# CaptainEven/DenseBox

Measured on AMD Instinct MI355X. Metric: training patches/sec (240x240), higher is better.
Workload: dtype f16; 1 GPU; full training step (fwd + fused dense loss w/ hard-negative mining + bwd + grad all-reduce + SGD) of DenseBoxLMLOC on 240x240 patches; net=DenseBoxLMLOC, batch_per_gpu=64, global_batch=64, patch=240x240, parallelism=dp1, half_neg=11, grad_finite=True

## Files before the change

densebox_amd/_lib.py:

```python
import ctypes as C
import os

_HERE = os.path.dirname(os.path.abspath(__file__))
LIB_PATH = os.environ.get('DBX_LIB') or os.path.join(_HERE, 'csrc', 'libdensebox_hip.so')

F16, BF16, F32 = 0, 1, 2
DTYPE_ID = {'f16': F16, 'bf16': BF16, 'f32': F32}
ESIZE = {F16: 2, BF16: 2, F32: 4}

EPI_BIAS, EPI_RELU, EPI_GATE, EPI_DROPMASK, EPI_ACCUM, EPI_F32_NCHW, EPI_DROPHASH = 1, 2, 4, 8, 16, 32, 64
CONV_WFRAG = 128
K_IGEMM, K_DMA, K_BAND, K_C64, K_C8, K_WS, K_P8 = 1, 2, 3, 4, 5, 6, 7


class View(C.Structure):
    _fields_ = [('ptr', C.c_void_p), ('n', C.c_int32), ('h', C.c_int32), ('w', C.c_int32),
                ('pad', C.c_int32), ('ld', C.c_int32), ('c_off', C.c_int32), ('c', C.c_int32)]


class ConvDesc(C.Structure):
    _fields_ = [('dtype', C.c_int32), ('kh', C.c_int32), ('kw', C.c_int32), ('cpad', C.c_int32),
                ('cin_pad', C.c_int32), ('cout_pad', C.c_int32), ('epilogue', C.c_int32), ('drop_seed', C.c_uint32)]


# ... 169 lines not shown
    'dbx_conv_forward': (C.c_int, [_PC, _PV, _VP, _VP, _PV, _PV, _VP, _I32, _VP]),
    'dbx_conv_plan': (C.c_int, [_PC, _PV, _PV, C.POINTER(ConvPlan)]),
    'dbx_conv_forward_split': (C.c_int, [_PC, _PV, _VP, _VP, _PV, _PV, _PV, _PV, _I32, _I32, _VP]),
    'dbx_heads_forward_fusable': (C.c_int, [_PC, _PV, _PV, C.POINTER(C.c_int32), _I32]),
    'dbx_heads_forward_fused_scratch_bytes': (_I64, [_I32, _I64]),
    'dbx_heads_forward_fused': (C.c_int, [_PC, _PV, _VP, _VP, _PV, _VP, _VP, C.POINTER(C.c_int32), _I32, _VP, _VP, _VP]),
    'dbx_heads_forward_fused_heads': (C.c_int, [_PC, _PV, _VP, _VP, _PV, _VP, _VP, C.POINTER(C.c_int32), _I32, C.POINTER(C.c_void_p), _VP, _VP]),
    'dbx_dp_unique_id': (C.c_int, [_VP]),
    'dbx_dp_init': (C.c_int, [_VP, _I32, _I32, C.POINTER(C.c_void_p)]),
    'dbx_dp_allreduce_sum_f32': (C.c_int, [_VP, _VP, _I64, _VP]),
    'dbx_dp_destroy': (C.c_int, [_VP]),
    'dbx_conv_dgrad_wgrad1_scratch_bytes': (_I64, []),
    'dbx_conv_dgrad_wgrad1_fusable': (C.c_int, [_PC, _PV, _PV, _PV]),
    'dbx_conv_dgrad_wgrad1': (C.c_int, [_PC, _PV, _VP, _PV, _PV, _I32, _VP, _VP, _VP, _I32, _VP]),
    'dbx_conv_pool_fusable': (C.c_int, [_PC, _PV, _PV]),
    'dbx_conv_forward_pool': (C.c_int, [_PC, _PV, _VP, _VP, _PV, _PV, _I32, _VP]),
    'dbx_conv_forward_pool_idx': (C.c_int, [_PC, _PV, _VP, _VP, _PV, _PV, _I32, _VP, _VP]),
    'dbx_pack_weight': (C.c_int, [_I32, _I32, _VP, _I32, _I32, _I32, _I32, _VP, _I32, _I32, _I32, _I32, _VP]),
    'dbx_fold_heads': (C.c_int, [_VP, _VP, _VP, _VP, _I32, _VP, _VP, _VP]),
    'dbx_fold_refine': (C.c_int, [_VP, _VP, _VP, _VP, _VP, _VP, _I32, _I32, _VP, _VP, _VP, _VP]),
    'dbx_refine_eval': (C.c_int, [_VP, _VP, _I32, _I32, _I32, _VP, _VP, _VP, _VP]),
    'dbx_refine_backward_scratch_bytes': (C.c_int64, [_I32, _I32, _I32]),
    'dbx_refine_backward': (C.c_int, [_VP, _VP, _VP, _I32, _I32, _I32, _VP, _VP, _VP, _VP, _VP, _VP, _I32, _VP, _VP, _VP, _VP, _VP, _VP, _VP, _VP, _VP, _VP, _VP, _VP, _VP, _VP]),
    'dbx_upsample_bilinear_nchw_f32': (C.c_int, [_VP, _I32, _I32, _I32, _VP, _I32, _I32, _VP]),
    'dbx_pack_multi': (C.c_int, [_I32, _VP, _I32, _I64, _VP]),
    'dbx_sgd_pack_step': (C.c_int, [_I32, _VP, _I32, _I64, _VP, _F, _F, _F, _I32, _VP]),
    'dbx_head2_dgrad': (C.c_int, [_I32, _PV, C.POINTER(C.c_void_p), C.POINTER(C.c_int32), _I32, _PV, _VP, _I32, _I32, C.c_uint32, _VP]),
    'dbx_head2_wgrad_scratch_bytes': (_I64, [_I32, _I32]),
    'dbx_head2_wgrad': (C.c_int, [_I32, _PV, _PV, C.POINTER(C.c_int32), _I32, C.POINTER(C.c_void_p), C.POINTER(C.c_void_p), _VP, _VP]),
    'dbx_head2_backward': (C.c_int, [_I32, _PV, _PV, C.POINTER(C.c_void_p), C.POINTER(C.c_int32), _I32, _PV, _VP, _I32, _I32, C.c_uint32,
                                     C.POINTER(C.c_void_p), C.POINTER(C.c_void_p), _VP, _VP]),
    'dbx_head2_backward_up': (C.c_int, [_I32, _PV, _PV, C.POINTER(C.c_void_p), C.POINTER(C.c_int32), _I32, _PV, _VP, _I32, _I32, C.c_uint32,
                                        C.POINTER(C.c_void_p), C.POINTER(C.c_void_p), _VP, _PV, _VP]),
    'dbx_perspective_matrix': (C.c_int, [_VP, _VP, _VP]),
    'dbx_warp_perspective_u8': (C.c_int, [_VP, _I32, _I32, _I32, _VP, _VP, _I32, _I32, _VP]),
    'dbx_warp_batch_workspace_bytes': (_I64, [_I32]),
    'dbx_warp_perspective_batch_u8': (C.c_int, [C.POINTER(WarpJob), _I32, _I32, _VP, _VP, _VP]),
    'dbx_plate_crops_batch': (C.c_int, [_VP, _I32, _I32, _VP, _I64, _I64, _VP, _I32, _I32, _I32, _VP, _VP, _VP, _VP]),
    'dbx_match_gt_batch': (C.c_int, [_VP, _I32, _I64, _VP, _VP, _I32, _I32, _VP, _I32, _VP, _VP, _I32, _D, _VP, _VP, _VP, _VP, _VP, _VP]),
    'dbx_eval_append': (C.c_int, [_VP, _I32, _I64, _VP, _VP, _I32, _I32, _VP, _VP, _VP, _VP, _I64, _VP, _VP]),
    'dbx_track_update_batch': (C.c_int, [_VP, _I32, _I64, _VP, _VP, _I32, _I32, _VP, _VP, _I32, _I32, _I32, _D, _I32, _D, _D, _D, _VP, _VP, _VP,
                                         _VP, _VP, _VP]),
    'dbx_track_append': (C.c_int, [_VP, _VP, _I32, _I32, _I32, _VP, _I64, _VP, _VP]),
    'dbx_crop_sharpness': (C.c_int, [_VP, _I64, _I32, _I32, _I32, _VP, _VP]),
    'dbx_track_gallery_update': (C.c_int, [_VP, _VP, _VP, _VP, _VP, _VP, _VP, _VP, _VP, _VP, _VP, _VP, _VP, _I32, _I32, _I32, _I32, _I32, _I32,
                                           _I32, _I32, _I64, _I32, _D, _I32, _VP]),
    'dbx_draw_overlay_batch': (C.c_int, [_VP, _I32, _I32, _I32, _I32, _VP, _I32, _I64, _VP, _VP, _I32, _VP, _VP, _VP, _I32, _I32,
                                         C.POINTER(OverlayStyle), _VP]),
    'dbx_overlay_font': (C.c_int, [_VP]),
    'dbx_overlay_label': (C.c_int, [_D, _I32, C.c_char_p, _I32]),
    'dbx_redact_batch': (C.c_int, [_VP, _I32, _I32, _I32, _I32, _VP, _I32, _I64, _VP, _VP, _I32, _VP, _I32, _I32, _I32,
                                   C.POINTER(RedactStyle), _VP]),
    'dbx_redact_host': (C.c_int, [_VP, _VP, _I32, _I32, _I32, _VP, _I32, _I32, _VP, _I32, _VP, _I32, C.POINTER(RedactStyle)]),
    'dbx_resize_batch_workspace_bytes': (_I64, [_I32]),
    'dbx_resize_cubic_batch_u8': (C.c_int, [C.POINTER(ResizeJob), _I32, _I32, _VP, _VP, _VP]),
    'dbx_nv12_to_rgb_batch': (C.c_int, [_VP, _I32, _I32, _I32, C.POINTER(Nv12Params), _VP]),
    'dbx_rgb_to_nv12_batch': (C.c_int, [_VP, _I32, _I32, _I32, C.POINTER(Nv12Params), _VP]),
    'dbx_nv12_host': (C.c_int, [C.POINTER(Nv12Frame), C.POINTER(Nv12Params), _I32]),
    'dbx_resize_batch_nv12_workspace_bytes': (_I64, [_I32]),
    'dbx_resize_cubic_batch_nv12': (C.c_int, [C.POINTER(ResizeJobNv12), _I32, C.POINTER(Nv12Params), _VP, _VP, _VP]),
    'dbx_patch_plan': (C.c_int, [C.POINTER(PatchPlanIO), _I32, _I32, _I32, _I32, _I32, _D, _D, _I32, _VP]),
    'dbx_patch_cut': (C.c_int, [_VP, _VP, _I32, _I32, _VP, _VP]),
    'dbx_patch_plan_host': (C.c_int, [_I32, _I32, _I32, _VP, _I32, _D, _D, _D, _I32, C.POINTER(PatchGeom)]),
    'dbx_patch_draw': (C.c_int, [_I64, _I64, _I32, _I32, _VP]),
    'dbx_patch_check_tables': (C.c_int, [_VP, _I32, _VP, _I32, _VP, _I32]),
    'dbx_patch_aug_plan': (C.c_int, [C.POINTER(PatchAugIO), C.POINTER(PatchAugCfg), _I32, _VP]),
# ... 104 lines not shown
```

densebox_amd/csrc/aux_ops.hip:

```cpp
#include "common.hpp"
#include <mutex>

static thread_local char g_err[512] = "";
void dbx_set_error(const char* fmt, ...) {
    va_list ap;
    va_start(ap, fmt);
    vsnprintf(g_err, sizeof(g_err), fmt, ap);
    va_end(ap);
}
extern "C" const char* dbx_last_error(void) { return g_err; }
extern "C" int dbx_version(void) { return DBX_ABI_VERSION; }
extern "C" int dbx_device_arch(int device) {
    hipDeviceProp_t p;
    if (hipGetDeviceProperties(&p, device) != hipSuccess) { dbx_set_error("hipGetDeviceProperties failed"); return DBX_ERR_HIP; }
    int arch = 0;
    const char* s = p.gcnArchName;
    if (s[0] == 'g' && s[1] == 'f' && s[2] == 'x') arch = (int)strtol(s + 3, nullptr, 16) == 0x950 ? 950 : (int)strtol(s + 3, nullptr, 10);
    return arch;
}

template <typename T> struct Vec { static constexpr int N = 16 / sizeof(T); };

template <typename T> __device__ __forceinline__ void load_vec(const T* p, float (&v)[16 / sizeof(T)]) {
    const u32x4 raw = *(const u32x4*)p;
// ... 1438 lines not shown
extern "C" int dbx_head2_backward_up_plan(int32_t dtype, const dbx_view* hid, const dbx_view* d_g44, const int32_t* k, int32_t nh,
                                          dbx_head2_up_plan_t* out) {
    if (!hid || !d_g44 || !k || !out) { dbx_set_error("head2_backward_up_plan: null argument"); return DBX_ERR_ARG; }
    if (dtype != DBX_F16 && dtype != DBX_BF16 && dtype != DBX_F32) { dbx_set_error("head2_backward_up_plan: unknown dtype"); return DBX_ERR_DTYPE; }
    DBX_REQUIRE(nh >= 1 && nh <= 4 && hid->c == 512 * nh && d_g44->n == hid->n && d_g44->c == hid->c,
                "head2_backward_up_plan: nh in 1..4, hid of 512*nh channels, d_g44 with the hidden map's batch and channels");
    for (int i = 0; i < nh; ++i) DBX_REQUIRE(k[i] >= 1 && k[i] <= 8, "head2_backward_up_plan: k in 1..8");
    *out = dbx_head2_up_plan_t{};
    float sy, sx;
    H2UPlan plan;
    if (!h2u_fused(dtype == DBX_F32 ? 4 : 2, hid, d_g44, sy, sx, plan)) return DBX_OK;
    out->fused = 1; out->halves = plan.halves;
    for (int i = 0; i < 2; ++i) {
        const H2UHalf& h = plan.h[i];
        out->half[i].px_lo = h.px_lo; out->half[i].px_n = h.px_n; out->half[i].own_lo = h.own_lo; out->half[i].own_hi = h.own_hi;
        out->half[i].ix_lo = h.ix_lo; out->half[i].ix_n = h.ix_n;
    }
    H2ULaunch l[4];
    out->launches = h2u_launches(k, nh, hid->n, plan.halves, l);
    for (int i = 0; i < out->launches; ++i) {
        out->launch[i].head0 = l[i].h0; out->launch[i].heads = l[i].nhl; out->launch[i].kj = l[i].kj; out->launch[i].groups = l[i].groups;
        out->launch[i].blocks = l[i].blocks;
    }
    return DBX_OK;
}
extern "C" int dbx_head2_backward_up(int32_t dtype, const dbx_view* d_out, const dbx_view* hid, const float* const* w2, const int32_t* k,
                                     int32_t nh, const dbx_view* d_hid, const uint8_t* dropmask, int32_t dropmask_ld, int32_t use_hash,
                                     uint32_t drop_seed, float* const* dw, float* const* db, void* scratch, const dbx_view* d_g44, void* stream) {
    if (!d_out || !hid || !w2 || !k || !d_hid || !dw || !scratch || !d_g44) { dbx_set_error("head2_backward_up: null argument"); return DBX_ERR_ARG; }
    DBX_DISPATCH_DTYPE(dtype, head2_backward_up_t, d_out, hid, w2, k, nh, d_hid, dropmask, dropmask_ld, use_hash, (unsigned)drop_seed, dw, db,
                       scratch, d_g44, (hipStream_t)stream);
}

struct PackJob { const float* src; void* dst; int co, ci, taps, mode; long long ktot; int cin_pad, row_off, k_off, rows_lim; };
template <typename T>
__global__ void pack_multi_kernel(const PackJob* __restrict__ jobs) {
    const PackJob j = jobs[blockIdx.y];
    const int total = j.co * j.ci * j.taps, taps = j.taps, ci = j.ci;
    T* wp = (T*)j.dst;
    const bool fwd = j.mode == 0 || j.mode == 4;
    const int rl = j.mode >= 4 ? (int)j.ktot : j.rows_lim;
    if (sizeof(T) == 2 && j.mode != 2 && (fwd ? ci : j.co) % 8 == 0 && (j.k_off & 7) == 0 && (j.cin_pad & 7) == 0 && taps <= 25) {
        __shared__ float tile[8][32 * 25];
        const int ot = (j.co + 7) / 8, ctn = (ci + 31) / 32, ntiles = ot * ctn, row_f = 32 * taps;
        for (int tl = blockIdx.x; tl < ntiles; tl += gridDim.x) {
            const int o0 = (tl / ctn) * 8, c0 = (tl % ctn) * 32;
            const int cw = min(32, ci - c0), ow = min(8, j.co - o0);
            __syncthreads();
            for (int e = threadIdx.x; e < 8 * row_f; e += blockDim.x) {
                const int r = e / row_f, f = e - r * row_f;
                tile[r][f] = (r < ow && f < cw * taps) ? j.src[((o0 + r) * ci + c0) * taps + f] : 0.f;
            }
            __syncthreads();
            const int nch = fwd ? 8 * taps * 4 : 32 * taps;
            for (int q = threadIdx.x; q < nch; q += blockDim.x) {
                int row, col, tap;
                float v[8];
                if (fwd) {
                    const int k8 = q & 3, t = (q >> 2) % taps, r = (q >> 2) / taps;
                    if (r >= ow || 8 * k8 >= cw) continue;
                    row = j.row_off + o0 + r; col = j.k_off + c0 + 8 * k8; tap = t;
#pragma unroll
                    for (int e = 0; e < 8; ++e) v[e] = tile[r][(8 * k8 + e) * taps + t];
                } else {
                    const int c = q % 32, t = q / 32;
                    if (c >= cw) continue;
// ... 358 lines not shown
```

densebox_amd/engine.py:

```python
import collections
import contextlib
import ctypes as C
import os
import weakref

import torch

from . import _lib
from ._lib import View, ConvDesc, check, ptr, stream_ptr

_BACKBONE = [('conv1_1_1', 3, 64), ('conv1_2_1', 64, 64), ('conv2_1_1', 64, 128), ('conv2_2_1', 128, 128),
             ('conv3_1_1', 128, 256), ('conv3_2_1', 256, 256), ('conv3_4_1', 256, 256),
             ('conv4_1_1', 256, 512), ('conv4_2_1', 512, 512), ('conv4_3_1', 512, 512), ('conv4_4_1', 512, 512)]

_HEADS = {
    'DenseBox': [('det', 1), ('loc', 4)],
    'DenseBoxLM': [('det', 1), ('loc', 4), ('landmark', 4)],
    'DenseBoxLMLOC': [('det', 1), ('loc', 4), ('landmark', 4), ('lmloc', 8)],
}


_FWD_IO = {'conv1_1_1': ('x0', 'a11'), 'conv1_2_1': ('a11', 'a12'), 'conv2_1_1': ('p1', 'a21'), 'conv2_2_1': ('a21', 'a22'),
           'conv3_1_1': ('p2', 'a31'), 'conv3_2_1': ('a31', 'a32'), 'conv3_4_1': ('a32', 'c34'), 'conv4_1_1': ('p3', 'a41'),
           'conv4_2_1': ('a41', 'a42'), 'conv4_3_1': ('a42', 'a43'), 'conv4_4_1': ('a43', 'a44')}
# ... 904 lines not shown
        for i, (stem, k) in enumerate(heads):
            slot[stem] = B['d_out'].view(P.crf * i, P.crf)
            src = override.get(stem)
            srcs.append(src if src is not None else gout(stem, k))
        if override or kind == 'DenseBox':
            check(L.dbx_nchw_to_framed_slots(dt, (C.c_void_p * nh)(*[t.data_ptr() for t in srcs]), (C.c_int32 * nh)(*[k for _, k in heads]), nh, P.crf,
                                             C.byref(B['d_out'].view()), s))
        else:
            for (stem, k), t in zip(heads, srcs):
                check(L.dbx_nchw_to_framed(dt, ptr(t), k, C.byref(slot[stem]), s))
        if kind != 'DenseBox' and not override:
            check(L.dbx_framed_add_ch(dt, C.byref(B['d_rf_in'].view()), 0, 4, C.byref(slot['landmark']), 0, s))
            check(L.dbx_framed_add_ch(dt, C.byref(B['d_rf_in'].view()), 4, 1, C.byref(slot['det']), 0, s))

        hv = B['hid'].view()
        need = L.dbx_head2_wgrad_scratch_bytes(nh, hv.n * hv.h)
        if getattr(self, '_h2_scratch', None) is None or self._h2_scratch.numel() < need:
            self._h2_scratch = torch.empty(int(need), dtype=torch.uint8, device=dev)
        dw2 = [new_grad('conv5_2_%s.weight' % st) for st, _ in heads]
        db2 = [new_grad('conv5_2_%s.bias' % st) for st, _ in heads]
        w2s = [self._param('conv5_2_%s.weight' % st).detach() for st, _ in heads]
        ks = (C.c_int32 * nh)(*[k for _, k in heads])
        h2_names = ['conv5_2_%s.weight' % st for st, _ in heads] + ['conv5_2_%s.bias' % st for st, _ in heads]
        mask_p = C.c_void_p(P.mask_buf.data_ptr()) if (P.drop_active and not P.drop_hash) else None
        hash_on, hash_seed = (1 if P.drop_hash else 0), (P.drop_seed if P.drop_hash else 0)
        lin = ('heads1', 'bwd_a') in M
        up_done = False
        gen = bool(getattr(P, 'heads_gen', False) and lin and side is None and mask_p is None)
        if gen and dt != _lib.F32:
            dhid_v = View(None, hv.n, hv.h, hv.w, 1, 512 * nh, 0, 512 * nh)
        else:
            dhid_v = self._d_hid(P).view()
        w2p = (C.c_void_p * nh)(*[w.data_ptr() for w in w2s])
        with self._timed(lambda: ('head2_backward_up_kernel<%s>' if up_done else 'head2_wgrad_kernel<%s>') % _TNAME[dt],
                         2.0 * hv.n * hv.h * hv.w * 512 * sum(k for _, k in heads) * (1 if side is not None else 2)):
            if side is not None:
                def run_h2():
                    check(L.dbx_head2_wgrad(dt, C.byref(B['d_out'].view()), C.byref(hv), ks, nh,
                                            (C.c_void_p * nh)(*[t.data_ptr() for t in dw2]), (C.c_void_p * nh)(*[t.data_ptr() for t in db2]),
                                            ptr(self._h2_scratch), stream_ptr()))
                    if sink is not None:
                        sink.ready(h2_names)
                on_side(run_h2)
                check(L.dbx_head2_dgrad(dt, C.byref(B['d_out'].view()), (C.c_void_p * nh)(*[w.data_ptr() for w in w2s]), ks, nh,
                                        C.byref(dhid_v), mask_p, 512 * nh, hash_on, hash_seed, s))
            elif lin:
                check(L.dbx_head2_backward_up(dt, C.byref(B['d_out'].view()), C.byref(hv), (C.c_void_p * nh)(*[w.data_ptr() for w in w2s]), ks, nh,
                                              C.byref(dhid_v), mask_p, 512 * nh, hash_on, hash_seed,
                                              (C.c_void_p * nh)(*[t.data_ptr() for t in dw2]), (C.c_void_p * nh)(*[t.data_ptr() for t in db2]),
                                              ptr(self._h2_scratch), C.byref(B['d_g44'].view()), s))
                up_done = True
                if gen and dt == _lib.F32:
                    bh = P.B['d_hid']
                    P.ws[bh.off:bh.off + bh.bytes].view(torch.float32).fill_(float('nan'))
            else:
                check(L.dbx_head2_backward(dt, C.byref(B['d_out'].view()), C.byref(hv), (C.c_void_p * nh)(*[w.data_ptr() for w in w2s]), ks, nh,
                                           C.byref(dhid_v), mask_p, 512 * nh, hash_on, hash_seed,
                                           (C.c_void_p * nh)(*[t.data_ptr() for t in dw2]), (C.c_void_p * nh)(*[t.data_ptr() for t in db2]),
                                           ptr(self._h2_scratch), s))
                if sink is not None:
                    sink.ready(h2_names)
        w1n = ['conv5_1_%s.weight' % st for st, _ in heads]
        b1n = ['conv5_1_%s.bias' % st for st, _ in heads]
        if sink is not None:
            dw1, db1 = sink.region(w1n).view(512 * nh, 768, 1, 1), sink.region(b1n)
        else:
            dw1 = torch.empty((512 * nh, 768, 1, 1), dtype=torch.float32, device=dev)
            db1 = torch.empty((512 * nh,), dtype=torch.float32, device=dev)
        c34 = B['fusion'].view(512, 256)
# ... 114 lines not shown
```

include/densebox_hip.h:

```cpp
#ifndef DENSEBOX_HIP_H
#define DENSEBOX_HIP_H

#include <stdint.h>

#ifdef __cplusplus
extern "C" {
#endif

enum dbx_status {
    DBX_OK = 0,
    DBX_ERR_ARG = -1,
    DBX_ERR_HIP = -2,
    DBX_ERR_DTYPE = -3
};

enum dbx_dtype { DBX_F16 = 0, DBX_BF16 = 1, DBX_F32 = 2 };

const char* dbx_last_error(void);
#define DBX_ABI_VERSION 13
int dbx_version(void);
int dbx_device_arch(int device);

typedef struct dbx_view {
    void*   ptr;
// ... 47 lines not shown
                                  const void* w2_frag, const float* bias2, const int32_t* k, int32_t nh, float* const* outs, void* scratch,
                                  void* stream);

int dbx_conv_forward_split(const dbx_conv_desc* d, const dbx_view* x, const void* w_packed, const float* bias,
                           const dbx_view* y, const dbx_view* gate, const dbx_view* y2, const dbx_view* gate2,
                           int32_t split_c, int32_t epilogue2, void* stream);

int dbx_conv_pool_fusable(const dbx_conv_desc* d, const dbx_view* x, const dbx_view* y);
int dbx_conv_forward_pool(const dbx_conv_desc* d, const dbx_view* x, const void* w_packed, const float* bias,
                          const dbx_view* y, const dbx_view* ypool, int32_t write_full, void* stream);
int dbx_conv_forward_pool_idx(const dbx_conv_desc* d, const dbx_view* x, const void* w_packed, const float* bias,
                              const dbx_view* y, const dbx_view* ypool, int32_t write_full, void* idx, void* stream);

int dbx_pack_weight(int32_t dtype, int32_t mode, const float* w_oihw, int32_t co, int32_t ci, int32_t kh, int32_t kw,
                    void* w_packed, int32_t rows_pad, int32_t cin_pad, int32_t row_off, int32_t k_off, void* stream);

int dbx_pack_multi(int32_t dtype, const void* jobs, int32_t count, int64_t max_elems, void* stream);

int dbx_sgd_pack_step(int32_t dtype, const void* jobs, int32_t count, int64_t max_elems, float* const* ptrs, float lr, float momentum,
                      float weight_decay, int32_t first_step, void* stream);

int dbx_head2_dgrad(int32_t dtype, const dbx_view* d_out, const float* const* w2, const int32_t* k, int32_t nh,
                    const dbx_view* d_hid, const uint8_t* dropmask, int32_t dropmask_ld, int32_t use_hash, uint32_t drop_seed,
                    void* stream);
int64_t dbx_head2_wgrad_scratch_bytes(int32_t nh, int32_t rows);
int dbx_head2_wgrad(int32_t dtype, const dbx_view* d_out, const dbx_view* hid, const int32_t* k, int32_t nh,
                    float* const* dw, float* const* db, void* scratch, void* stream);
int dbx_head2_backward(int32_t dtype, const dbx_view* d_out, const dbx_view* hid, const float* const* w2, const int32_t* k,
                       int32_t nh, const dbx_view* d_hid, const uint8_t* dropmask, int32_t dropmask_ld, int32_t use_hash,
                       uint32_t drop_seed, float* const* dw, float* const* db, void* scratch, void* stream);
int dbx_head2_backward_up(int32_t dtype, const dbx_view* d_out, const dbx_view* hid, const float* const* w2, const int32_t* k,
                          int32_t nh, const dbx_view* d_hid, const uint8_t* dropmask, int32_t dropmask_ld, int32_t use_hash,
                          uint32_t drop_seed, float* const* dw, float* const* db, void* scratch, const dbx_view* d_g44, void* stream);
int dbx_conv_wgrad_pool_dz_ok(int32_t dtype, const dbx_view* dz, const dbx_view* x, int32_t kh, int32_t kw);
int dbx_conv_wgrad_pool_dz(int32_t dtype, const dbx_view* dy, const void* idx, int32_t idx_channels, const dbx_view* dz, const dbx_view* x,
                           int32_t kh, int32_t kw, int32_t cpad, int32_t co, int32_t ci, float* dw_oihw, float* db, void* scratch,
                           int32_t accumulate, int32_t write_dz, void* stream);
int dbx_head2_backward_up_fused(int32_t dtype, const dbx_view* hid, const dbx_view* d_g44);
typedef struct dbx_head2_up_half { int32_t px_lo, px_n, own_lo, own_hi, ix_lo, ix_n; } dbx_head2_up_half;
typedef struct dbx_head2_up_launch { int32_t head0, heads, kj, groups, blocks; } dbx_head2_up_launch;
typedef struct dbx_head2_up_plan_t {
    int32_t fused, halves;
    dbx_head2_up_half half[2];
    int32_t launches;
    dbx_head2_up_launch launch[4];
} dbx_head2_up_plan_t;
int dbx_head2_backward_up_plan(int32_t dtype, const dbx_view* hid, const dbx_view* d_g44, const int32_t* k, int32_t nh,
                               dbx_head2_up_plan_t* out);
int dbx_heads1_wgrad_gen_ok(int32_t dtype, const dbx_view* x, int32_t nh);
int dbx_heads1_wgrad_gen(int32_t dtype, const dbx_view* d_out, const dbx_view* x, const float* const* w2, const int32_t* k, int32_t nh,
                         int32_t use_hash, uint32_t drop_seed, int32_t ci, float* dw_oihw, int32_t dw_ci_total, int32_t dw_ci_off,
                         float* db, void* scratch, void* stream);
int dbx_heads1_dgrad_gen(int32_t dtype, const dbx_view* d_out, const float* const* w2, const int32_t* k, int32_t nh, int32_t use_hash,
                         uint32_t drop_seed, const void* w1t_frag, const dbx_view* y, const dbx_view* gate, void* stream);

int dbx_fold_heads(const float* w2, const float* b2, const float* w1, const float* b1, int32_t k, float* w_out,
                   float* b_out, void* stream);
int dbx_fold_refine(const float* w1, const float* b1, const float* w2, const float* b2, const float* w3, const float* b3,
                    int32_t ci, int32_t cm, float* w_out, float* b_out, float* v_out, void* stream);
int dbx_refine_eval(const float* landmark_nchw, const float* score_nchw, int32_t n, int32_t h, int32_t w, const float* w_fold,
                    const float* b_fold, float* out_small, void* stream);
int dbx_upsample_bilinear_nchw_f32(const float* x, int32_t planes, int32_t hi, int32_t wi, float* y, int32_t ho, int32_t wo,
                                   void* stream);
int64_t dbx_refine_backward_scratch_bytes(int32_t n, int32_t h, int32_t w);
int dbx_refine_backward(const float* d_refine, const float* landmark, const float* score, int32_t n, int32_t h, int32_t w,
                        const float* w1, const float* b1, const float* w2, const float* b2, const float* w3, const float* b3,
// ... 406 lines not shown
```

Before: 7288 patches/s.

## Split head2 backward for loc heads into zero-skipping wgrad and fused dg44 generation

Adds two kernels for the trailing localization heads. One computes the head2 weight gradient and skips pixel batches whose output gradient is all zero, which hard-negative mining makes sparse. The other generates the upsampled hidden gradient directly from d_out and the head weights, skipping rows that are all zero. Leading non-loc heads still go through the existing backward_up path. The change adds two extra launches and more code paths, and how much work it saves depends on how sparse the loc-head gradient is.

```diff
diff --git a/densebox_amd/_lib.py b/densebox_amd/_lib.py
--- a/densebox_amd/_lib.py
+++ b/densebox_amd/_lib.py
@@ -225,6 +225,8 @@
                                      C.POINTER(C.c_void_p), C.POINTER(C.c_void_p), _VP, _VP]),
     'dbx_head2_backward_up': (C.c_int, [_I32, _PV, _PV, C.POINTER(C.c_void_p), C.POINTER(C.c_int32), _I32, _PV, _VP, _I32, _I32, C.c_uint32,
                                         C.POINTER(C.c_void_p), C.POINTER(C.c_void_p), _VP, _PV, _VP]),
+    'dbx_head2_wgrad_skip': (C.c_int, [_I32, _PV, _PV, C.POINTER(C.c_int32), _I32, _I32, _I32, C.POINTER(C.c_void_p), C.POINTER(C.c_void_p), _VP, _VP]),
+    'dbx_head2_dg44_gen': (C.c_int, [_I32, _PV, C.POINTER(C.c_void_p), C.POINTER(C.c_int32), _I32, _I32, _I32, _PV, _VP, _I32, C.c_uint32, _PV, _VP]),
     'dbx_perspective_matrix': (C.c_int, [_VP, _VP, _VP]),
     'dbx_warp_perspective_u8': (C.c_int, [_VP, _I32, _I32, _I32, _VP, _VP, _I32, _I32, _VP]),
     'dbx_warp_batch_workspace_bytes': (_I64, [_I32]),
diff --git a/densebox_amd/csrc/aux_ops.hip b/densebox_amd/csrc/aux_ops.hip
--- a/densebox_amd/csrc/aux_ops.hip
+++ b/densebox_amd/csrc/aux_ops.hip
@@ -1494,6 +1494,426 @@
                        scratch, d_g44, (hipStream_t)stream);
 }
 
+template <typename T>
+__global__ __launch_bounds__(256) void head2_wgrad_skip_kernel(FrameGeo dout, FrameGeo hid, int nh, int head0, int heads, int slot, int ppb, int nblk,
+                                                               float* __restrict__ partial, float* __restrict__ bpartial) {
+    static_assert(sizeof(T) == 2, "16-bit element types");
+    constexpr int V = 8, B = 8;
+    typedef float f32x2 __attribute__((ext_vector_type(2)));
+    const int blk = blockIdx.x / heads, hd = head0 + (blockIdx.x - blk * heads);
+    const int grp = __builtin_amdgcn_readfirstlane((int)(threadIdx.x >> 6)), lane = threadIdx.x & 63, c0 = lane * V;
+    f32x2 acc[8][V / 2];
+    float bs[8];
+#pragma unroll
+    for (int j = 0; j < 8; ++j) {
+        bs[j] = 0.f;
+#pragma unroll
+        for (int i = 0; i < V / 2; ++i) acc[j][i] = (f32x2){0.f, 0.f};
+    }
+    const int npix = hid.n * hid.h * hid.w;
+    const int per = (npix + nblk - 1) / nblk;
+    const int p0 = blk * per, p1 = p0 + per < npix ? p0 + per : npix;
+    if (p0 + grp < p1) {
+        const int cnt = (p1 - p0 - grp + ppb - 1) / ppb;
+        const unsigned HW = (unsigned)(hid.h * hid.w), W = (unsigned)hid.w;
+        const unsigned n0 = (unsigned)(p0 + grp) / HW, rem0 = (unsigned)(p0 + grp) - n0 * HW;
+        const char* const hbase = hid.base + (size_t)(hd * 512 + c0) * sizeof(T);
+        const int nchunks = (cnt + 63) / 64;
+        u32x4 gnx;
+        unsigned honx_lo, honx_hi;
+        auto gfetch = [&](int chunk) {
+            int idx = chunk * 64 + lane;
+            idx = idx < cnt ? idx : cnt - 1;
+            const unsigned q = rem0 + (unsigned)idx * (unsigned)ppb;
+            const unsigned dn = q / HW, r = q - dn * HW, y = r / W, x = r - y * W;
+            gnx = *(const u32x4*)((const T*)dout.base + geo_pix(dout, (int)(n0 + dn), (int)y, (int)x) + hd * slot);
+            const size_t ho = geo_pix(hid, (int)(n0 + dn), (int)y, (int)x) * sizeof(T);
+            honx_lo = (unsigned)ho; honx_hi = (unsigned)(ho >> 32);
+        };
+        gfetch(0);
+        for (int c = 0; c < nchunks; ++c) {
+            const bool in = c * 64 + lane < cnt;
+            const u32x4 graw = in ? gnx : (u32x4){0u, 0u, 0u, 0u};
+            const unsigned ho_lo = honx_lo, ho_hi = honx_hi;
+            gfetch(c + 1 < nchunks ? c + 1 : c);
+            unsigned long long todo = __ballot(((graw.x | graw.y | graw.z | graw.w) & 0x7fff7fffu) != 0u);
+            if (todo == 0ull) continue;
+            float gf[8];
+            {
+                const T* ge = (const T*)&graw;
+#pragma unroll
+                for (int j = 0; j < 8; ++j) gf[j] = to_f32(ge[j]);
+            }
+            auto next_batch = [&]() {
+                if (todo == 0ull) return -1;
+                const int b = __builtin_ctzll(todo) >> 3;
+                todo &= ~(0xffull << (8 * b));
+                return b;
+            };
+            auto hload = [&](int b, u32x4 (&h)[B]) {
+#pragma unroll
+                for (int d = 0; d < B; ++d) {
+                    const unsigned lo = (unsigned)__builtin_amdgcn_readlane((int)ho_lo, b * 8 + d), hi = (unsigned)__builtin_amdgcn_readlane((int)ho_hi, b * 8 + d);
+                    h[d] = *(const u32x4*)(hbase + (((size_t)hi << 32) | lo));
+                }
+            };
+            auto accumulate = [&](int b, const u32x4 (&hr)[B]) {
+#pragma unroll
+                for (int d = 0; d < B; ++d) {
+                    float gj[8], h[V];
+                    const T* he = (const T*)&hr[d];
+#pragma unroll
+                    for (int j = 0; j < 8; ++j) gj[j] = __builtin_bit_cast(float, __builtin_amdgcn_readlane(__builtin_bit_cast(int, gf[j]), b * 8 + d));
+#pragma unroll
+                    for (int i = 0; i < V; ++i) h[i] = to_f32(he[i]);
+#pragma unroll
+                    for (int j = 0; j < 8; ++j) {
+                        bs[j] += gj[j];
+                        const f32x2 g2 = {gj[j], gj[j]};
+#pragma unroll
+                        for (int i = 0; i < V / 2; ++i) acc[j][i] = g2 * (f32x2){h[2 * i], h[2 * i + 1]} + acc[j][i];
+                    }
+                }
+            };
+            u32x4 ha[B], hb[B];
+            int b0 = next_batch();
+            hload(b0, ha);
+            for (;;) {
+                const int b1 = next_batch();
+                hload(b1 >= 0 ? b1 : b0, hb);
+                __builtin_amdgcn_sched_barrier(0);
+                accumulate(b0, ha);
+                if (b1 < 0) break;
+                const int b2 = next_batch();
+                hload(b2 >= 0 ? b2 : b1, ha);
+                __builtin_amdgcn_sched_barrier(0);
+                accumulate(b1, hb);
+                if (b2 < 0) break;
+                b0 = b2;
+            }
+        }
+    }
+    __shared__ float red[256 * V];
+    float* P = partial + ((size_t)blk * nh + hd) * 8 * 512;
+    for (int j = 0; j < 8; ++j) {
+        __syncthreads();
+#pragma unroll
+        for (int i = 0; i < V; ++i) red[threadIdx.x * V + i] = acc[j][i >> 1][i & 1];
+        __syncthreads();
+        if (threadIdx.x < 64) {
+            float o[V];
+#pragma unroll
+            for (int i = 0; i < V; ++i) o[i] = 0.f;
+            for (int q = 0; q < ppb; ++q)
+#pragma unroll
+                for (int i = 0; i < V; ++i) o[i] += red[(q * 64 + lane) * V + i];
+#pragma unroll
+            for (int i = 0; i < V; ++i) P[(size_t)j * 512 + c0 + i] = o[i];
+        }
+    }
+    __syncthreads();
+    if (lane == 0) {
+#pragma unroll
+        for (int j = 0; j < 8; ++j) red[grp * 8 + j] = bs[j];
+    }
+    __syncthreads();
+    if (threadIdx.x < 8) {
+        float o = 0.f;
+        for (int q = 0; q < ppb; ++q) o += red[q * 8 + threadIdx.x];
+        bpartial[(size_t)blk * 32 + hd * 8 + threadIdx.x] = o;
+    }
+}
+template <typename T>
+static int head2_wgrad_skip_t(const dbx_view* dout, const dbx_view* hid, const int32_t* k, int nh, int head0, int heads, float* const* dw, float* const* db,
+                              void* scratch, hipStream_t s) {
+    if constexpr (sizeof(T) != 2) {
+        dbx_set_error("head2_wgrad_skip: 16-bit types only (dbx_head2_wgrad takes fp32)");
+        return DBX_ERR_DTYPE;
+    } else {
+        VIEW_VEC_CHECK(T, hid, "head2_wgrad_skip hid");
+        DBX_REQUIRE(nh >= 1 && nh <= 4 && hid->c == 512 * nh && dout->c % nh == 0 && dout->c / nh >= 8, "head2_wgrad_skip: nh in 1..4, hid of 512*nh channels, d_out of nh slots >= 8 channels");
+        DBX_REQUIRE(dout->n == hid->n && dout->h == hid->h && dout->w == hid->w && hid->n >= 1 && hid->h >= 1 && hid->w >= 1, "head2_wgrad_skip: shape mismatch");
+        DBX_REQUIRE((long long)hid->n * hid->h * hid->w < (1ll << 30), "head2_wgrad_skip: fewer than 2**30 pixels (32-bit pixel arithmetic)");
+        DBX_REQUIRE(((size_t)dout->ptr % 16) == 0 && (dout->ld * sizeof(T)) % 16 == 0 && (dout->c_off * sizeof(T)) % 16 == 0 &&
+                        ((dout->c / nh) * sizeof(T)) % 16 == 0, "head2_wgrad_skip: d_out alignment");
+        Head2Out o;
+        for (int i = 0; i < 4; ++i) {
+            o.dw[i] = i < nh ? dw[i] : nullptr; o.db[i] = (i < nh && db) ? db[i] : nullptr; o.k[i] = i < nh ? k[i] : 0;
+            if (i < nh) DBX_REQUIRE(k[i] >= 1 && k[i] <= 8 && dw[i], "head2_wgrad_skip: k in 1..8");
+            if (i < head0 || i >= head0 + heads) o.k[i] = 0;
+        }
+        DBX_REQUIRE(head0 >= 0 && heads >= 1 && head0 + heads <= nh, "head2_wgrad_skip: heads [head0, head0 + heads) inside [0, nh)");
+        const int lph_all = 64 * nh;
+        const int ppb = (lph_all <= 256 ? 256 : 512) / lph_all;
+        const int blocks = head2_wgrad_blocks(hid->n * hid->h);
+        float* partial = (float*)scratch;
+        float* bpartial = partial + (size_t)blocks * nh * 8 * 512;
+        hipLaunchKernelGGL(head2_wgrad_skip_kernel<T>, dim3(blocks * heads), dim3(64 * ppb), 0, s, make_geo<T>(dout), make_geo<T>(hid), nh, head0, heads, dout->c / nh,
+                           ppb, blocks, partial, bpartial);
+        DBX_LAUNCH_CHECK();
+        for (int i = 0; i < 4; ++i) { o.poff[i] = 0; o.boff[i] = 0; o.nblk[i] = (i >= head0 && i < head0 + heads) ? blocks : 0; o.nhl[i] = nh; o.hl[i] = i; }
+        const int total = nh * 8 * 512 + nh * 8;
+        hipLaunchKernelGGL(head2_wgrad_reduce_kernel, dim3((total + 63) / 64), dim3(1024), 0, s, partial, bpartial, blocks, nh, o);
+        DBX_LAUNCH_CHECK();
+        return DBX_OK;
+    }
+}
+extern "C" int dbx_head2_wgrad_skip(int32_t dtype, const dbx_view* d_out, const dbx_view* hid, const int32_t* k, int32_t nh, int32_t head0, int32_t heads,
+                                    float* const* dw, float* const* db, void* scratch, void* stream) {
+    if (!d_out || !hid || !k || !dw || !scratch) { dbx_set_error("head2_wgrad_skip: null argument"); return DBX_ERR_ARG; }
+    DBX_DISPATCH_DTYPE(dtype, head2_wgrad_skip_t, d_out, hid, k, nh, head0, heads, dw, db, scratch, (hipStream_t)stream);
+}
+
+#define H2G_CB 64
+template <typename T, int KJ>
+__device__ __forceinline__ void head2_dg44_gen_body(const FrameGeo& dout, const FrameGeo& dg, int H, int W, int img, int hd, int cbase, int slot,
+                                                    int use_hash, unsigned drop_seed, float sy, float* s_v, const float* s_w,
+                                                    unsigned long long rowmask, int tlo0, int tcnt0, const float (&tcf0)[6], int tlo1, int tcnt1,
+                                                    const float (&tcf1)[6]) {
+    constexpr int V = 8, CB = H2G_CB, LPP = CB / V, PL = 256 / LPP, NP = 64 / PL, NT = 6;
+    typedef float f32x2 __attribute__((ext_vector_type(2)));
+    const int tid = threadIdx.x, ch = tid % LPP, pl = tid / LPP, c0 = cbase + ch * V;
+    const float* const wl = s_w + ch * V;
+    int pxs[NP];
+#pragma unroll
+    for (int u = 0; u < NP; ++u) pxs[u] = pl + PL * u < W ? pl + PL * u : W - 1;
+    auto next_row = [&](int from) {
+        const unsigned long long m = from < 64 ? rowmask >> from : 0ull;
+        return m ? from + (int)__builtin_ctzll(m) : H;
+    };
+    u32x4 gq[2][NP];
+    auto gfetch = [&](int d, int oy) {
+#pragma unroll
+        for (int u = 0; u < NP; ++u) gq[d][u] = *(const u32x4*)((const T*)dout.base + geo_pix(dout, img, oy, pxs[u]) + hd * slot);
+    };
+    f32x2 va[NP][V / 2], vb[NP][V / 2];
+#pragma unroll
+    for (int u = 0; u < NP; ++u)
+#pragma unroll
+        for (int i = 0; i < V / 2; ++i) va[u][i] = vb[u][i] = (f32x2){0.f, 0.f};
+    bool vaf = false, vbf = false;
+    int par = 0;
+    T* const gbase = (T*)dg.base + hd * 512 + cbase;
+    auto finalize = [&](int iy, const f32x2 (&v)[NP][V / 2], bool has) {
+        if (has) {
+            float* buf = s_v + par * (64 * CB);
+#pragma unroll
+            for (int u = 0; u < NP; ++u)
+                if (pl + PL * u < W) {
+                    *(f32x4*)&buf[(pl + PL * u) * CB + ch * V] = (f32x4){v[u][0].x, v[u][0].y, v[u][1].x, v[u][1].y};
+                    *(f32x4*)&buf[(pl + PL * u) * CB + ch * V + 4] = (f32x4){v[u][2].x, v[u][2].y, v[u][3].x, v[u][3].y};
+                }
+            __syncthreads();
+            par ^= 1;
+#pragma unroll
+            for (int r = 0; r < 2; ++r) {
+                const int q = tid + 256 * r;
+                if (q < dg.w * (CB / 4)) {
+                    const int ix = q / (CB / 4), tq = q % (CB / 4);
+                    const int tlo = r ? tlo1 : tlo0, tcnt = r ? tcnt1 : tcnt0;
+                    f32x4 c = {0.f, 0.f, 0.f, 0.f};
+#pragma unroll
+                    for (int t = 0; t < NT; ++t) {
+                        const int o = tlo + t < W ? tlo + t : W - 1;
+                        const f32x4 a = *(const f32x4*)&buf[o * CB + tq * 4];
+                        const float cf = r ? tcf1[t] : tcf0[t];
+                        if (t < tcnt) { c.x = fmaf(cf, a.x, c.x); c.y = fmaf(cf, a.y, c.y); c.z = fmaf(cf, a.z, c.z); c.w = fmaf(cf, a.w, c.w); }
+                    }
+                    u32x2 raw;
+                    T* e = (T*)&raw;
+                    e[0] = from_f32<T>(c.x); e[1] = from_f32<T>(c.y); e[2] = from_f32<T>(c.z); e[3] = from_f32<T>(c.w);
+                    *(u32x2*)(gbase + geo_pix(dg, img, iy, ix) + tq * 4) = raw;
+                }
+            }
+        } else {
+#pragma unroll
+            for (int r = 0; r < 2; ++r) {
+                const int q = tid + 256 * r;
+                if (q < dg.w * (CB / 4)) *(u32x2*)(gbase + geo_pix(dg, img, iy, q / (CB / 4)) + (q % (CB / 4)) * 4) = (u32x2){0u, 0u};
+            }
+        }
+    };
+    int nr = next_row(0), nr1 = next_row(nr + 1);
+    gfetch(0, nr < H ? nr : 0);
+    gfetch(1, nr1 < H ? nr1 : 0);
+    int cur = 0;
+    for (int oy = 0; oy < H; ++oy) {
+        int y0, y1; float ly0, ly1;
+        bilin_coef(oy, sy, dg.h, y0, y1, ly0, ly1);
+        while (y0 > cur) {
+            finalize(cur, va, vaf);
+#pragma unroll
+            for (int u = 0; u < NP; ++u)
+#pragma unroll
+                for (int i = 0; i < V / 2; ++i) { va[u][i] = vb[u][i]; vb[u][i] = (f32x2){0.f, 0.f}; }
+            vaf = vbf; vbf = false;
+            ++cur;
+        }
+        if (oy != nr) continue;
+        u32x4 graw[NP];
+#pragma unroll
+        for (int u = 0; u < NP; ++u) { graw[u] = gq[0][u]; gq[0][u] = gq[1][u]; }
+        nr = nr1;
+        nr1 = next_row(nr1 + 1);
+        gfetch(1, nr1 < H ? nr1 : oy);
+        const float wa = (y0 == cur ? ly0 : 0.f) + (y1 == cur ? ly1 : 0.f);
+        const float wb = (y0 == cur + 1 ? ly0 : 0.f) + (y1 == cur + 1 ? ly1 : 0.f);
+        const f32x2 wa2 = {wa, wa}, wb2 = {wb, wb};
+        const unsigned pc0 = (unsigned)(((long long)img * H + oy) * W);
+        f32x2 o2[NP][V / 2];
+#pragma unroll
+        for (int u = 0; u < NP; ++u)
+#pragma unroll
+            for (int i = 0; i < V / 2; ++i) o2[u][i] = (f32x2){0.f, 0.f};
+        asm volatile("" ::: "memory");
+#pragma unroll
+        for (int j = 0; j < KJ; ++j) {
+            const f32x4 a = *(const f32x4*)&wl[j * CB], c = *(const f32x4*)&wl[j * CB + 4];
+            const f32x2 wr[V / 2] = {(f32x2){a.x, a.y}, (f32x2){a.z, a.w}, (f32x2){c.x, c.y}, (f32x2){c.z, c.w}};
+#pragma unroll
+            for (int u = 0; u < NP; ++u) {
+                const float gj = to_f32(((const T*)&graw[u])[j]);
+                const f32x2 g2 = {gj, gj};
+#pragma unroll
+                for (int i = 0; i < V / 2; ++i) o2[u][i] = g2 * wr[i] + o2[u][i];
+            }
+            if (j % 2 == 1) __builtin_amdgcn_sched_barrier(0);
+        }
+#pragma unroll
+        for (int u = 0; u < NP; ++u) {
+            float o[V];
+#pragma unroll
+            for (int i = 0; i < V / 2; ++i) { o[2 * i] = o2[u][i].x; o[2 * i + 1] = o2[u][i].y; }
+            if (use_hash) {
+                const unsigned kb8 = dbx_drop_hash32(drop_seed, pc0 + (unsigned)pxs[u], (unsigned)(hd * 512 + c0) >> 5) >> ((unsigned)c0 & 31u);
+#pragma unroll
+                for (int i = 0; i < V; ++i)
+                    o[i] = __builtin_bit_cast(float, __builtin_bit_cast(int, o[i]) & __builtin_amdgcn_sbfe((int)kb8, i, 1));
+            }
+#pragma unroll
+            for (int i = 0; i < V / 2; ++i) {
+                const f32x2 dv = {to_f32(from_f32<T>(o[2 * i])), to_f32(from_f32<T>(o[2 * i + 1]))};
+                va[u][i] = wa2 * dv + va[u][i]; vb[u][i] = wb2 * dv + vb[u][i];
+            }
+        }
+        vaf = vbf = true;
+    }
+    finalize(cur, va, vaf);
+    if (cur + 1 < dg.h) finalize(cur + 1, vb, vbf);
+}
+template <typename T>
+__global__ __launch_bounds__(256) void head2_dg44_gen_kernel(FrameGeo dout, FrameGeo dg, int H, int W, int head0, int heads, int slot, Head2Args ha, int use_hash,
+                                                             unsigned drop_seed, float sy, float sx) {
+    static_assert(sizeof(T) == 2, "16-bit element types");
+    constexpr int CB = H2G_CB, NT = 6;
+    __shared__ int s_x0[64], s_lo[32], s_hi[32];
+    __shared__ unsigned s_rowmask[2];
+    __shared__ float s_l0[64], s_l1[64];
+    __shared__ __attribute__((aligned(16))) float s_v[2 * 64 * CB], s_w[8 * CB];
+    int b = blockIdx.x;
+    const int hd = head0 + b % heads; b /= heads;
+    const int cbase = (b % (512 / CB)) * CB, img = b / (512 / CB);
+    const int tid = threadIdx.x;
+    int k = ha.k[0];
+    const float* wp = ha.w2[0];
+#pragma unroll
+    for (int hh = 1; hh < 4; ++hh)
+        if (hd == hh) { k = ha.k[hh]; wp = ha.w2[hh]; }
+    if (tid < 32) { s_lo[tid] = W; s_hi[tid] = -1; }
+    if (tid < 2) s_rowmask[tid] = 0u;
+    if (tid < 8 * CB / 4) {
+        const int j = tid / (CB / 4), c4 = (tid % (CB / 4)) * 4;
+        const f32x4 w = *(const f32x4*)(wp + (size_t)(j < k ? j : k - 1) * 512 + cbase + c4);
+        const float dscale = use_hash ? 2.f : 1.f;
+        f32x4 o = {to_f32(from_f32<T>(w.x)) * dscale, to_f32(from_f32<T>(w.y)) * dscale, to_f32(from_f32<T>(w.z)) * dscale, to_f32(from_f32<T>(w.w)) * dscale};
+        if (j >= k) o = (f32x4){0.f, 0.f, 0.f, 0.f};
+        *(f32x4*)&s_w[j * CB + c4] = o;
+    }
+    __syncthreads();
+    if (tid < W) {
+        int x0, x1; float lx0, lx1;
+        bilin_coef(tid, sx, dg.w, x0, x1, lx0, lx1);
+        s_x0[tid] = x0; s_l0[tid] = x1 == x0 ? lx0 + lx1 : lx0; s_l1[tid] = x1 == x0 ? 0.f : lx1;
+        atomicMin(&s_lo[x0], tid); atomicMax(&s_hi[x0], tid);
+        if (x0 + 1 < dg.w) { atomicMin(&s_lo[x0 + 1], tid); atomicMax(&s_hi[x0 + 1], tid); }
+    }
+    for (int p0 = tid; p0 < H * W; p0 += 1024) {
+        u32x4 g[4];
+#pragma unroll
+        for (int t = 0; t < 4; ++t) {
+            const int p = p0 + 256 * t < H * W ? p0 + 256 * t : 0;
+            const int y = p / W, x = p - y * W;
+            g[t] = *(const u32x4*)((const T*)dout.base + geo_pix(dout, img, y, x) + hd * slot);
+        }
+#pragma unroll
+        for (int t = 0; t < 4; ++t) {
+            const int p = p0 + 256 * t;
+            if (p < H * W && ((g[t].x | g[t].y | g[t].z | g[t].w) & 0x7fff7fffu) != 0u) atomicOr(&s_rowmask[(p / W) >> 5], 1u << ((p / W) & 31));
+        }
+    }
+    __syncthreads();
+    int tlo[2], tcnt[2];
+    float tcf[2][NT];
+#pragma unroll
+    for (int r = 0; r < 2; ++r) {
+        const int q = tid + 256 * r, ix = q / (CB / 4);
+        tlo[r] = 0; tcnt[r] = 0;
+#pragma unroll
+        for (int t = 0; t < NT; ++t) tcf[r][t] = 0.f;
+        if (ix < dg.w) {
+            const int lo = s_lo[ix];
+            tlo[r] = lo < W ? lo : 0; tcnt[r] = s_hi[ix] - lo + 1;
+#pragma unroll
+            for (int t = 0; t < NT; ++t) {
+                const int ox = lo + t < W ? lo + t : W - 1;
+                tcf[r][t] = s_x0[ox] == ix ? s_l0[ox] : s_l1[ox];
+            }
+        }
+    }
+    const unsigned long long rowmask = (unsigned long long)(unsigned)__builtin_amdgcn_readfirstlane((int)s_rowmask[0]) |
+                                       ((unsigned long long)(unsigned)__builtin_amdgcn_readfirstlane((int)s_rowmask[1]) << 32);
+#define H2G_BODY(KJ) head2_dg44_gen_body<T, KJ>(dout, dg, H, W, img, hd, cbase, slot, use_hash, drop_seed, sy, s_v, s_w, rowmask, tlo[0], tcnt[0], tcf[0], \
+                                                tlo[1], tcnt[1], tcf[1])
+    if (k <= 1) H2G_BODY(1); else if (k <= 2) H2G_BODY(2); else if (k <= 4) H2G_BODY(4); else H2G_BODY(8);
+#undef H2G_BODY
+}
+template <typename T>
+static int head2_dg44_gen_t(const dbx_view* dout, const float* const* w2, const int32_t* k, int nh, int head0, int heads, const dbx_view* hid, const uint8_t* mask,
+                            int use_hash, unsigned drop_seed, const dbx_view* dg, hipStream_t s) {
+    if constexpr (sizeof(T) != 2) {
+        dbx_set_error("head2_dg44_gen: 16-bit types only");
+        return DBX_ERR_DTYPE;
+    } else {
+        VIEW_VEC_CHECK(T, dg, "head2_dg44_gen d_g44");
+        DBX_REQUIRE(!mask, "head2_dg44_gen: a byte dropout mask needs the hidden gradient's stored form (hash / no dropout only, as dbx_head2_backward_up without d_hid)");
+        DBX_REQUIRE(nh >= 1 && nh <= 4 && hid->c == 512 * nh && dout->c % nh == 0 && dout->c / nh >= 8, "head2_dg44_gen: nh in 1..4, a hidden map of 512*nh channels, d_out of nh slots >= 8 channels");
+        DBX_REQUIRE(dg->n == hid->n && dg->c == hid->c && dout->n == hid->n && dout->h == hid->h && dout->w == hid->w, "head2_dg44_gen: shape mismatch");
+        DBX_REQUIRE(head0 >= 0 && heads >= 1 && head0 + heads <= nh, "head2_dg44_gen: heads [head0, head0 + heads) inside [0, nh)");
+        DBX_REQUIRE(((size_t)dout->ptr % 16) == 0 && (dout->ld * sizeof(T)) % 16 == 0 && (dout->c_off * sizeof(T)) % 16 == 0 &&
+                        ((dout->c / nh) * sizeof(T)) % 16 == 0, "head2_dg44_gen: d_out alignment");
+        float sy, sx;
+        H2UPlan plan;
+        DBX_REQUIRE(h2u_fused(sizeof(T), hid, dg, sy, sx, plan), "head2_dg44_gen: needs the maps of the one-pass form (dbx_head2_backward_up_fused)");
+        DBX_REQUIRE(hid->h <= 64 && hid->w <= 64 && dg->w <= 32 && (long long)hid->n * nh * (512 / H2G_CB) < (1ll << 31),
+                    "head2_dg44_gen: a hidden map of up to 64 x 64 pixels");
+        Head2Args ha;
+        ha.nh = nh; ha.slot = dout->c / nh;
+        for (int i = 0; i < 4; ++i) {
+            ha.w2[i] = i < nh ? w2[i] : nullptr; ha.k[i] = i < nh ? k[i] : 0;
+            if (i < nh) DBX_REQUIRE(k[i] >= 1 && k[i] <= 8 && w2[i] && ((size_t)w2[i] % 16) == 0, "head2_dg44_gen: k in 1..8, 16-byte aligned weights");
+        }
+        hipLaunchKernelGGL(head2_dg44_gen_kernel<T>, dim3((unsigned)(hid->n * heads * (512 / H2G_CB))), dim3(256), 0, s, make_geo<T>(dout), make_geo<T>(dg),
+                           hid->h, hid->w, head0, heads, dout->c / nh, ha, use_hash, drop_seed, sy, sx);
+        DBX_LAUNCH_CHECK();
+        return DBX_OK;
+    }
+}
+extern "C" int dbx_head2_dg44_gen(int32_t dtype, const dbx_view* d_out, const float* const* w2, const int32_t* k, int32_t nh, int32_t head0, int32_t heads, const dbx_view* hid,
+                                  const uint8_t* dropmask, int32_t use_hash, uint32_t drop_seed, const dbx_view* d_g44, void* stream) {
+    if (!d_out || !w2 || !k || !hid || !d_g44) { dbx_set_error("head2_dg44_gen: null argument"); return DBX_ERR_ARG; }
+    DBX_DISPATCH_DTYPE(dtype, head2_dg44_gen_t, d_out, w2, k, nh, head0, heads, hid, dropmask, use_hash, (unsigned)drop_seed, d_g44, (hipStream_t)stream);
+}
+
 struct PackJob { const float* src; void* dst; int co, ci, taps, mode; long long ktot; int cin_pad, row_off, k_off, rows_lim; };
 template <typename T>
 __global__ void pack_multi_kernel(const PackJob* __restrict__ jobs) {
diff --git a/densebox_amd/engine.py b/densebox_amd/engine.py
--- a/densebox_amd/engine.py
+++ b/densebox_amd/engine.py
@@ -960,9 +960,34 @@
         else:
             dhid_v = self._d_hid(P).view()
         w2p = (C.c_void_p * nh)(*[w.data_ptr() for w in w2s])
-        with self._timed(lambda: ('head2_backward_up_kernel<%s>' if up_done else 'head2_wgrad_kernel<%s>') % _TNAME[dt],
-                         2.0 * hv.n * hv.h * hv.w * 512 * sum(k for _, k in heads) * (1 if side is not None else 2)):
-            if side is not None:
+        lead = nh
+        if gen and dt != _lib.F32 and hv.h <= 64:
+            mode = os.environ.get('DBX_HEAD2_SPLIT', '1')
+            if mode == '2':
+                lead = 0
+            elif mode != '0':
+                while lead > 0 and heads[lead - 1][0] in ('loc', 'lmloc'):
+                    lead -= 1
+        if lead < nh:
+            dwp, dbp = (C.c_void_p * nh)(*[t.data_ptr() for t in dw2]), (C.c_void_p * nh)(*[t.data_ptr() for t in db2])
+            if lead > 0:
+                with self._timed('head2_backward_up_kernel<%s>' % _TNAME[dt], 4.0 * hv.n * hv.h * hv.w * 512 * sum(k for _, k in heads[:lead])):
+                    check(L.dbx_head2_backward_up(dt, C.byref(B['d_out'].view(0, P.crf * lead)), C.byref(B['hid'].view(0, 512 * lead)), w2p,
+                                                  (C.c_int32 * lead)(*[k for _, k in heads[:lead]]), lead,
+                                                  C.byref(View(None, hv.n, hv.h, hv.w, 1, 512 * nh, 0, 512 * lead)), None, 512 * nh, hash_on, hash_seed,
+                                                  dwp, dbp, ptr(self._h2_scratch), C.byref(B['d_g44'].view(0, 512 * lead)), s))
+            tail_flops = 2.0 * hv.n * hv.h * hv.w * 512 * sum(k for _, k in heads[lead:])
+            with self._timed('head2_wgrad_skip_kernel<%s>' % _TNAME[dt], tail_flops):
+                check(L.dbx_head2_wgrad_skip(dt, C.byref(B['d_out'].view()), C.byref(hv), ks, nh, lead, nh - lead, dwp, dbp, ptr(self._h2_scratch), s))
+            with self._timed('head2_dg44_gen_kernel<%s>' % _TNAME[dt], tail_flops):
+                check(L.dbx_head2_dg44_gen(dt, C.byref(B['d_out'].view()), w2p, ks, nh, lead, nh - lead, C.byref(hv), None, hash_on, hash_seed,
+                                           C.byref(B['d_g44'].view()), s))
+            up_done = True
+        with _NOT_TIMED if lead < nh else self._timed(lambda: ('head2_backward_up_kernel<%s>' if up_done else 'head2_wgrad_kernel<%s>') % _TNAME[dt],
+                                                      2.0 * hv.n * hv.h * hv.w * 512 * sum(k for _, k in heads) * (1 if side is not None else 2)):
+            if lead < nh:
+                pass
+            elif side is not None:
                 def run_h2():
                     check(L.dbx_head2_wgrad(dt, C.byref(B['d_out'].view()), C.byref(hv), ks, nh,
                                             (C.c_void_p * nh)(*[t.data_ptr() for t in dw2]), (C.c_void_p * nh)(*[t.data_ptr() for t in db2]),
diff --git a/include/densebox_hip.h b/include/densebox_hip.h
--- a/include/densebox_hip.h
+++ b/include/densebox_hip.h
@@ -103,6 +103,10 @@
 int dbx_head2_backward_up(int32_t dtype, const dbx_view* d_out, const dbx_view* hid, const float* const* w2, const int32_t* k,
                           int32_t nh, const dbx_view* d_hid, const uint8_t* dropmask, int32_t dropmask_ld, int32_t use_hash,
                           uint32_t drop_seed, float* const* dw, float* const* db, void* scratch, const dbx_view* d_g44, void* stream);
+int dbx_head2_wgrad_skip(int32_t dtype, const dbx_view* d_out, const dbx_view* hid, const int32_t* k, int32_t nh, int32_t head0, int32_t heads,
+                         float* const* dw, float* const* db, void* scratch, void* stream);
+int dbx_head2_dg44_gen(int32_t dtype, const dbx_view* d_out, const float* const* w2, const int32_t* k, int32_t nh, int32_t head0, int32_t heads,
+                       const dbx_view* hid, const uint8_t* dropmask, int32_t use_hash, uint32_t drop_seed, const dbx_view* d_g44, void* stream);
 int dbx_conv_wgrad_pool_dz_ok(int32_t dtype, const dbx_view* dz, const dbx_view* x, int32_t kh, int32_t kw);
 int dbx_conv_wgrad_pool_dz(int32_t dtype, const dbx_view* dy, const void* idx, int32_t idx_channels, const dbx_view* dz, const dbx_view* x,
                            int32_t kh, int32_t kw, int32_t cpad, int32_t co, int32_t ci, float* dw_oihw, float* db, void* scratch,
```

New measurement: 7337 patches/s (median of 6 runs). Within noise of the previous version (+0.7%).
